# Coder-Yu/SELFRec

Hardware: NVIDIA H100
Metric: XSimGCL yelp2018 train steps/sec (higher is better)
Workload: dtype f32

## Files before the change

include/selfrec_b200.h:

```cpp
#ifndef SELFREC_B200_H
#define SELFREC_B200_H

#include <stdint.h>

#ifdef __cplusplus
extern "C" {
#endif

#define SRB_OK 0
#define SRB_ERR_ARG (-1)
#define SRB_ERR_CUDA (-2)
#define SRB_ERR_STATE (-3)

const char* srb_last_error(void);
int srb_version(void);
int64_t srb_launch_count(void);
int srb_device_ok(void);

#define SRB_HUB_CHUNK 2048
#define SRB_HUB_MIN_NNZ 4096
#define SRB_HUB_WARP_SEG 256
typedef struct srb_hub_split {
  int32_t n_rows;
  int32_t n_work;
  const int32_t* first;
  const int32_t* work;
  float* part;
  const int32_t* seg;
  const int32_t* seg_cnt;
  const int32_t* order_cta;
  const int32_t* order_warp;
  int32_t n_cta;
  int32_t n_warp;
} srb_hub_split;

typedef struct srb_spmm_desc {
  const int32_t* rowptr;
  const int32_t* colidx;
  const float* vals;
  int32_t n_rows;
  int32_t n_cols;
  int32_t d;
  const int32_t* row_order;
  int32_t n_long_rows;
  int32_t n_vlong_rows;
  srb_hub_split hub;
  const int32_t* n_vlong_dev;
  const uint32_t* col_mask;
  const float* X;
// ... 3 lines not shown
  int32_t noise_mode;
  const float* noise;
  float eps;
  uint64_t philox_seed;
  uint64_t philox_offset;
  const int32_t* philox_step_dev;
  const float* sum_in;
  float* sum_out;
  float sum_scale;
  float* adam_p;
  float* adam_m;
  float* adam_v;
  const float* adam_scalars;
  double beta1, beta2;
  float adam_eps;
} srb_spmm_desc;

int srb_spmm_csr(const srb_spmm_desc* desc, void* stream);
int srb_spmm_epilogue_rows(const srb_spmm_desc* desc, void* stream);

typedef struct srb_encoder_desc {
  const int32_t* rowptr;
  const int32_t* colidx;
  const float* vals;
  const int32_t* row_order;
  int32_t n_long_rows;
  int32_t n_vlong_rows;
  srb_hub_split hub;
  int32_t n;
  int32_t d;
// ... 5 lines not shown
  float eps;
  uint64_t philox_seed;
  uint64_t philox_offset;
  const int32_t* philox_step_dev;
  const int32_t* last_rows;
  int32_t n_last_rows;
  const int32_t* last_rows_nv_dev;
  srb_hub_split last_rows_hub;
  float* last_rows_out;
  const float* E0;
  float* final_out;
  float* cl_out;
  float* work0;
  float* work1;
  const float* x1;
} srb_encoder_desc;

int srb_encoder_forward(const srb_encoder_desc* desc, void* stream);

typedef struct srb_bpr_desc {
  const float* emb;
  const float* l2_emb;
  int32_t n_users;
  int32_t d;
  const int32_t* u_idx;
  const int32_t* i_idx;
  const int32_t* j_idx;
  const int32_t* b_dev;
  int32_t b;
  float emb_scale;
// ... 138 lines not shown

int srb_rank_hit_masks(const int32_t* topk_ids, int32_t n_q, int32_t k, const int32_t* users,
                       const int32_t* test_ptr, const int32_t* test_idx, uint64_t* hit_mask,
                       void* stream);

enum { SRB_MODEL_MF = 0, SRB_MODEL_LIGHTGCN = 1, SRB_MODEL_SIMGCL = 2, SRB_MODEL_XSIMGCL = 3, SRB_MODEL_SGL = 4 };

typedef struct srb_graph_csr {
  const int32_t* rowptr;
  const int32_t* colidx;
  const float* vals;
  const int32_t* row_order;
  int32_t n_long_rows;
  int32_t n_vlong_rows;
  srb_hub_split hub;
} srb_graph_csr;

typedef struct srb_step_desc {
  int32_t model;
  int32_t n_users, n_items, d, n_layers;
  int32_t batch_cap;
  int32_t layer_cl;
  float eps, tau, cl_rate;
  float reg;
  double lr, beta1, beta2;
  float adam_eps;
  float l2_div;
  int32_t noise_mode;
  const float* noise;
  uint64_t philox_seed;
// ... 118 lines not shown
```

selfrec_b200/_lib.py:

```python
import ctypes as C
import os

HERE = os.path.dirname(os.path.abspath(__file__))
LIB_PATH = os.path.join(HERE, "libselfrec_b200.so")

c_i32p = C.POINTER(C.c_int32)
c_f32p = C.POINTER(C.c_float)
c_u32p = C.POINTER(C.c_uint32)
c_i64p = C.POINTER(C.c_int64)
VP = C.c_void_p


class SrbError(RuntimeError):
    pass


class HubSplit(C.Structure):
    _fields_ = [("n_rows", C.c_int32), ("n_work", C.c_int32), ("first", VP), ("work", VP), ("part", VP), ("seg", VP), ("seg_cnt", VP),
                ("order_cta", VP), ("order_warp", VP), ("n_cta", C.c_int32), ("n_warp", C.c_int32)]


HUB_CHUNK = 2048
HUB_MIN_NNZ = 4096
HUB_WARP_SEG = 256


class SpmmDesc(C.Structure):
    _fields_ = [
        ("rowptr", VP), ("colidx", VP), ("vals", VP),
        ("n_rows", C.c_int32), ("n_cols", C.c_int32), ("d", C.c_int32),
        ("row_order", VP), ("n_long_rows", C.c_int32), ("n_vlong_rows", C.c_int32), ("hub", HubSplit), ("n_vlong_dev", VP), ("col_mask", VP), ("X", VP), ("Y", VP), ("extra", VP), ("extra_scale", C.c_float),
        ("noise_mode", C.c_int32), ("noise", VP), ("eps", C.c_float),
        ("philox_seed", C.c_uint64), ("philox_offset", C.c_uint64), ("philox_step_dev", VP),
        ("sum_in", VP), ("sum_out", VP), ("sum_scale", C.c_float),
        ("adam_p", VP), ("adam_m", VP), ("adam_v", VP), ("adam_scalars", VP),
        ("beta1", C.c_double), ("beta2", C.c_double), ("adam_eps", C.c_float),
    ]


class EncoderDesc(C.Structure):
    _fields_ = [
        ("rowptr", VP), ("colidx", VP), ("vals", VP), ("row_order", VP), ("n_long_rows", C.c_int32),
        ("n_vlong_rows", C.c_int32), ("hub", HubSplit), ("n", C.c_int32), ("d", C.c_int32), ("n_layers", C.c_int32), ("include_ego", C.c_int32),
        ("layer_cl", C.c_int32), ("noise_mode", C.c_int32), ("noise", VP), ("eps", C.c_float),
        ("philox_seed", C.c_uint64), ("philox_offset", C.c_uint64), ("philox_step_dev", VP),
        ("last_rows", VP), ("n_last_rows", C.c_int32), ("last_rows_nv_dev", VP), ("last_rows_hub", HubSplit), ("last_rows_out", VP),
        ("E0", VP), ("final_out", VP), ("cl_out", VP), ("work0", VP), ("work1", VP), ("x1", VP),
    ]


class ScatterSeg(C.Structure):
    _fields_ = [("src", VP), ("rows", VP), ("n_dev", VP), ("n", C.c_int32), ("row_off", C.c_int32), ("scale", C.c_float)]


class BprDesc(C.Structure):
    _fields_ = [
        ("emb", VP), ("l2_emb", VP), ("n_users", C.c_int32), ("d", C.c_int32),
        ("u_idx", VP), ("i_idx", VP), ("j_idx", VP), ("b_dev", VP), ("b", C.c_int32),
        ("emb_scale", C.c_float), ("reg", C.c_float), ("l2_terms", C.c_int32), ("l2_div", C.c_float),
        ("grad_scale", C.c_float), ("losses", VP), ("g_emb", VP), ("g_l2", VP), ("scratch", VP),
    ]

# ... 12 lines not shown
        ("prob", InfoNceProblem * 4), ("workspace", VP), ("workspace_bytes", C.c_int64),
    ]


class TopkDesc(C.Structure):
    _fields_ = [
        ("user_emb", VP), ("item_emb", VP), ("n_items", C.c_int32), ("d", C.c_int32),
        ("users", VP), ("n_q", C.c_int32), ("rated_ptr", VP), ("rated_idx", VP), ("k", C.c_int32),
        ("out_ids", VP), ("out_scores", VP), ("impl", C.c_int32), ("workspace", VP),
        ("workspace_bytes", C.c_int64),
    ]


class GraphCsr(C.Structure):
    _fields_ = [("rowptr", VP), ("colidx", VP), ("vals", VP), ("row_order", VP), ("n_long_rows", C.c_int32), ("n_vlong_rows", C.c_int32),
                ("hub", HubSplit)]


class GraphAssembleDesc(C.Structure):
    _fields_ = [
        ("n_users", C.c_int32), ("n_items", C.c_int32), ("nnz", C.c_int64), ("ui_ptr", VP), ("ui_col", VP), ("ui_val", VP),
        ("iu_ptr", VP), ("iu_col", VP), ("iu_perm", VP), ("keep_flags", VP), ("keep_idx", VP), ("n_keep", C.c_int64),
        ("reset_weights", C.c_int32), ("dinv_table", VP), ("dinv_table_n", C.c_int32), ("rowptr", VP), ("colidx", VP),
        ("vals", VP), ("dinv", VP), ("out_cap", C.c_int64), ("nnz_out", VP), ("workspace", VP), ("workspace_bytes", C.c_int64),
    ]


class StepDesc(C.Structure):
    _fields_ = [
        ("model", C.c_int32), ("n_users", C.c_int32), ("n_items", C.c_int32), ("d", C.c_int32),
        ("n_layers", C.c_int32), ("batch_cap", C.c_int32), ("layer_cl", C.c_int32),
# ... 141 lines not shown
```

selfrec_b200/csrc/engine.cu:

```cuda
#include <stdlib.h>
#include <algorithm>
#include <mutex>
#include "spmm_args.cuh"

namespace srb {

static bool pdl_enabled() {
  static const bool on = [] {
    const char* e = getenv("SRB_PDL");
    return !(e && e[0] == '0');
  }();
  return on;
}

static thread_local bool t_pdl = false;
bool pdl_active() { return t_pdl; }

struct PdlScope {
  PdlScope() { t_pdl = pdl_enabled(); }
  ~PdlScope() { t_pdl = false; }
};

struct Ws {
  float* final_;
// ... 352 lines not shown
static ScatterSeg seg(const float* src, const int32_t* rows, const int32_t* n_dev, int n, int row_off, float scale) {
  ScatterSeg g = {src, rows, n_dev, n, row_off, scale};
  return g;
}

static int encoder(const srb_step_desc* s, const Ws& w, const srb_graph_csr* g, bool include_ego, int noise_mode, int view,
                   int layer_cl, float* final_out, float* cl_out, cudaStream_t st, const float* x1 = nullptr) {
  srb_encoder_desc e = {};
  e.rowptr = g->rowptr;
  e.colidx = g->colidx;
  e.vals = g->vals;
  e.row_order = g->row_order;
  e.n_long_rows = g->n_long_rows;
  e.n_vlong_rows = g->n_vlong_rows;
  e.hub = g->hub;
  e.n = s->n_users + s->n_items;
  e.d = s->d;
  e.n_layers = s->n_layers;
  e.include_ego = include_ego;
  e.layer_cl = layer_cl;
  e.noise_mode = noise_mode;
  if (noise_mode == 1) e.noise = s->noise + (size_t)view * s->n_layers * e.n * e.d;
  e.eps = s->eps;
  e.philox_seed = s->philox_seed;
  e.philox_offset = noise_offset(view, 0);
  e.philox_step_dev = s->step_dev;
  e.E0 = s->params;
  if (cl_out && layer_cl == s->n_layers) {
    e.final_out = final_out;
  } else {
// ... 152 lines not shown
```

selfrec_b200/csrc/spmm.cu:

```cuda
#include "spmm_args.cuh"

namespace srb {

__device__ __forceinline__ void st4_cs(float* p, const float4& v, int stream) {
  if (stream) __stcs(reinterpret_cast<float4*>(p), v);
  else st4(p, v);
}

__device__ __forceinline__ void st4_peer(float* p, const float4& v, int mc) {
  if (mc) asm volatile("multimem.st.weak.global.v4.f32 [%0], {%1, %2, %3, %4};" ::"l"(p), "f"(v.x), "f"(v.y), "f"(v.z), "f"(v.w) : "memory");
  else st4(p, v);
}

__device__ __forceinline__ float4 ldg4_if(const float* p, bool pred) {
  float4 r = f4_zero();
  asm("{\n\t.reg .pred q;\n\tsetp.ne.b32 q, %5, 0;\n\t@q ld.global.nc.v4.f32 {%0, %1, %2, %3}, [%4];\n\t}"
      : "+f"(r.x), "+f"(r.y), "+f"(r.z), "+f"(r.w)
      : "l"(p), "r"((int)pred));
  return r;
}

template <int D>
__device__ __forceinline__ void spmm_epilogue(const SpmmArgs& a, int row, int gl, float4 acc0, float4 acc1, bool valid) {
  constexpr int LPR = D / 8;
  constexpr int HALF = D / 2;
  {
    if (a.stage_peer[0]) {
      if (!valid) return;
      int o = 0;
#pragma unroll 1
      while (row >= a.stage_bounds[o + 1]) ++o;
      float* dst = a.stage_peer[o] + ((size_t)a.stage_rank * a.stage_cap + (row - a.stage_bounds[o])) * D + gl * 4;
      st4(dst, acc0);
      st4(dst + HALF, acc1);
// ... 93 lines not shown
  p4.F = p4.F - step_size * (m.F / (sqrtf(v4.F) / bc2_sqrt + a.aeps));
        SRB_ADAM1(x) SRB_ADAM1(y) SRB_ADAM1(z) SRB_ADAM1(w)
#undef SRB_ADAM1
        st4(a.ap + o2, p4);
        st4_cs(a.am + o2, m, a.stream);
        st4_cs(a.av + o2, v4, a.stream);
        if (a.world > 0 && a.peer_p[0]) {
#pragma unroll 1
          for (int g = 0; g < a.world; ++g) st4_peer(a.peer_p[g] + o2, p4, a.peer_mc);
        }
      }
    }
  }
}

template <int D, bool MASKED>
__device__ __forceinline__ void spmm_gather(const SpmmArgs& a, int p, int end, int stride, int gl, float4& acc0, float4& acc1) {
  constexpr int LPR = D / 8;
  constexpr int HALF = D / 2;
  constexpr int SB = LPR < 4 ? LPR : 4;
  constexpr bool masked = MASKED;
  const int lane = threadIdx.x & 31;
  const int gbase = lane - gl;
  int c = 0;
  float v = 0.f;
  bool hit = false;
  if (p + gl < end) {
    c = a.stream ? __ldcs(a.colidx + p + gl) : __ldg(a.colidx + p + gl);
    v = a.stream ? __ldcs(a.vals + p + gl) : __ldg(a.vals + p + gl);
    if (masked) hit = (__ldg(a.col_mask + (c >> 5)) >> (c & 31)) & 1u;
  }
  while (__any_sync(SRB_FULL_MASK, p < end)) {
    int cn = 0;
    float vn = 0.f;
    bool hitn = false;
    if (p + stride + gl < end) {
      cn = a.stream ? __ldcs(a.colidx + p + stride + gl) : __ldg(a.colidx + p + stride + gl);
      vn = a.stream ? __ldcs(a.vals + p + stride + gl) : __ldg(a.vals + p + stride + gl);
      if (masked) hitn = (__ldg(a.col_mask + (cn >> 5)) >> (cn & 31)) & 1u;
    }
    if (!masked) {
#pragma unroll
      for (int j0 = 0; j0 < LPR; j0 += SB) {
        if (j0 > 0 && !__any_sync(SRB_FULL_MASK, p + j0 < end)) break;
        float vv[SB];
        float4 x0[SB], x1[SB];
#pragma unroll
        for (int j = 0; j < SB; ++j) {
          const int cc = __shfl_sync(SRB_FULL_MASK, c, j0 + j, LPR);
          vv[j] = __shfl_sync(SRB_FULL_MASK, v, j0 + j, LPR);
          const float* xr = a.X + (size_t)cc * D + gl * 4;
          x0[j] = ldg4(xr);
          x1[j] = ldg4(xr + HALF);
        }
// ... 16 lines not shown
          gm &= gm - 1;
          const int cc = __shfl_sync(SRB_FULL_MASK, c, gbase + src);
          const float vs = __shfl_sync(SRB_FULL_MASK, v, gbase + src);
          vv[j] = live ? vs : 0.f;
          const float* xr = a.X + (size_t)cc * D + gl * 4;
          x0[j] = ldg4_if(xr, live);
          x1[j] = ldg4_if(xr + HALF, live);
        }
#pragma unroll
        for (int j = 0; j < SB; ++j) {
          acc0 = f4_fma(vv[j], x0[j], acc0);
          acc1 = f4_fma(vv[j], x1[j], acc1);
        }
      }
    }
    c = cn;
    v = vn;
    hit = hitn;
    p += stride;
  }
}

__device__ __forceinline__ void xor_reduce_groups(float4& acc0, float4& acc1, int lpr) {
  for (int o = lpr; o < 32; o <<= 1) {
    acc0.x += __shfl_xor_sync(SRB_FULL_MASK, acc0.x, o);
    acc0.y += __shfl_xor_sync(SRB_FULL_MASK, acc0.y, o);
    acc0.z += __shfl_xor_sync(SRB_FULL_MASK, acc0.z, o);
    acc0.w += __shfl_xor_sync(SRB_FULL_MASK, acc0.w, o);
    acc1.x += __shfl_xor_sync(SRB_FULL_MASK, acc1.x, o);
    acc1.y += __shfl_xor_sync(SRB_FULL_MASK, acc1.y, o);
    acc1.z += __shfl_xor_sync(SRB_FULL_MASK, acc1.z, o);
    acc1.w += __shfl_xor_sync(SRB_FULL_MASK, acc1.w, o);
  }
}

template <int D, bool MASKED>
__global__ void __launch_bounds__(256) spmm_hub_kernel(const SpmmArgs a) {
  constexpr int LPR = D / 8;
  const int lane = threadIdx.x & 31;
  const int wib = threadIdx.x >> 5;
  const int grp = lane / LPR;
  const int gl = lane % LPR;
  pdl_wait();
  pdl_trigger();
  const int n_work = a.seg ? a.n_cta : (a.n_vlong_dev ? min(a.n_vlong_dev[4], a.n_work) : a.n_work);
  __shared__ float4 part[8][2][LPR];
  for (int k = blockIdx.x; k < n_work; k += gridDim.x) {
    int w = k, beg, end;
    if (a.seg) {
      w = __ldg(a.order_cta + k);
      beg = __ldg(a.seg + 2 * w);
      end = __ldg(a.seg + 2 * w + 1);
    } else {
      const int row = __ldg(a.hub_work + 2 * w);
      const int ci = __ldg(a.hub_work + 2 * w + 1);
      const int rbeg = __ldg(a.rowptr + row), rend = __ldg(a.rowptr + row + 1);
      beg = min(rend, rbeg + ci * SRB_HUB_CHUNK);
      end = min(rend, beg + SRB_HUB_CHUNK);
    }
    const int per = ((end - beg + 255) / 256) * 32;
    const int wbeg = beg + wib * per;
    const int wend = min(end, wbeg + per);
    float4 acc0 = f4_zero(), acc1 = f4_zero();
    spmm_gather<D, MASKED>(a, wbeg + grp * LPR, wend, 32, gl, acc0, acc1);
    xor_reduce_groups(acc0, acc1, LPR);
    if (grp == 0) {
      part[wib][0][gl] = acc0;
      part[wib][1][gl] = acc1;
    }
    __syncthreads();
    if (wib == 0 && grp == 0) {
      acc0 = f4_zero();
      acc1 = f4_zero();
#pragma unroll
      for (int q = 0; q < 8; ++q) {
        acc0 = f4_add(acc0, part[q][0][gl]);
        acc1 = f4_add(acc1, part[q][1][gl]);
      }
      float* dst = a.hub_part + (size_t)w * D + gl * 4;
// ... 6 lines not shown

template <int D, bool MASKED>
__global__ void __launch_bounds__(256) spmm_seg_warp_kernel(const SpmmArgs a) {
  constexpr int LPR = D / 8;
  const int lane = threadIdx.x & 31;
  const int grp = lane / LPR;
  const int gl = lane % LPR;
  const int warp0 = (blockIdx.x * blockDim.x + threadIdx.x) >> 5;
  const int nwarps = (gridDim.x * blockDim.x) >> 5;
  pdl_wait();
  pdl_trigger();
  for (int k = warp0; k < a.n_warp; k += nwarps) {
    const int w = __ldg(a.order_warp + k);
    const int beg = __ldg(a.seg + 2 * w), end = __ldg(a.seg + 2 * w + 1);
    float4 acc0 = f4_zero(), acc1 = f4_zero();
    spmm_gather<D, MASKED>(a, beg + grp * LPR, end, 32, gl, acc0, acc1);
    xor_reduce_groups(acc0, acc1, LPR);
    if (grp == 0) {
      float* dst = a.hub_part + (size_t)w * D + gl * 4;
      st4(dst, acc0);
      st4(dst + D / 2, acc1);
    }
  }
}

template <int D>
__global__ void __launch_bounds__(256) spmm_hub_finish_kernel(const SpmmArgs a) {
  constexpr int LPR = D / 8;
  constexpr int RPW = 32 / LPR;
  const int lane = threadIdx.x & 31;
  const int grp = lane / LPR;
// ... 8 lines not shown
    const int row = __ldg(a.row_order + vr);
    const int first = __ldg(a.hub_first + vr);
    const int deg = __ldg(a.rowptr + row + 1) - __ldg(a.rowptr + row);
    const int nch = a.seg ? __ldg(a.seg_cnt + vr) : (deg + SRB_HUB_CHUNK - 1) / SRB_HUB_CHUNK;
    float4 acc0 = f4_zero(), acc1 = f4_zero();
    for (int c = grp; c < nch; c += RPW) {
      const float* src = a.hub_part + (size_t)(first + c) * D + gl * 4;
      acc0 = f4_add(acc0, *reinterpret_cast<const float4*>(src));
      acc1 = f4_add(acc1, *reinterpret_cast<const float4*>(src + D / 2));
    }
    xor_reduce_groups(acc0, acc1, LPR);
    spmm_epilogue<D>(a, row, gl, acc0, acc1, grp == 0);
  }
}

template <int D, bool MASKED>
__global__ void __launch_bounds__(256) spmm_csr_kernel(const SpmmArgs a) {
  constexpr int LPR = D / 8;
  constexpr int RPW = 32 / LPR;
  const int lane = threadIdx.x & 31;
  const int wib = threadIdx.x >> 5;
  const int grp = lane / LPR;
  const int gl = lane % LPR;
  const int warp0 = (blockIdx.x * blockDim.x + threadIdx.x) >> 5;
  const int nwarps = (gridDim.x * blockDim.x) >> 5;

  pdl_wait();
  pdl_trigger();
  peer_wait(a.ps);
  int n_vlong = a.n_vlong, n_long = a.n_long, n_short = a.n_rows - a.n_huge - a.n_vlong - a.n_long;
  const int32_t* ro_v = a.row_order ? a.row_order + a.n_huge : nullptr;
  const int32_t* ro_l = a.row_order ? ro_v + n_vlong : nullptr;
// ... 3 lines not shown
    n_vlong = min(a.n_vlong_dev[1], a.n_rows);
    n_long = min(a.n_vlong_dev[2], a.n_rows);
    n_short = min(a.n_vlong_dev[3], a.n_rows);
    ro_v = a.row_order + a.n_rows;
    ro_l = a.row_order + 2 * a.n_rows;
    ro_s = a.row_order + 3 * a.n_rows;
  }
  __shared__ float4 part[8][2][LPR];
  for (int vr = blockIdx.x; vr < n_vlong; vr += gridDim.x) {
    const int row = ro_v ? __ldg(ro_v + vr) : vr;
    const int beg = __ldg(a.rowptr + row);
    const int end = __ldg(a.rowptr + row + 1);
    const int per = ((end - beg + 255) / 256) * 32;
    const int wbeg = beg + wib * per;
    const int wend = min(end, wbeg + per);
    float4 acc0 = f4_zero(), acc1 = f4_zero();
    spmm_gather<D, MASKED>(a, wbeg + grp * LPR, wend, 32, gl, acc0, acc1);
    xor_reduce_groups(acc0, acc1, LPR);
    if (grp == 0) {
      part[wib][0][gl] = acc0;
      part[wib][1][gl] = acc1;
    }
    __syncthreads();
    if (wib == 0) {
      acc0 = f4_zero();
      acc1 = f4_zero();
#pragma unroll
      for (int w = 0; w < 8; ++w) {
        acc0 = f4_add(acc0, part[w][0][gl]);
        acc1 = f4_add(acc1, part[w][1][gl]);
      }
      spmm_epilogue<D>(a, row, gl, acc0, acc1, grp == 0);
    }
    __syncthreads();
  }

  const int n_items = n_long + (n_short + RPW - 1) / RPW;
  for (int item = warp0; item < n_items; item += nwarps) {
    const bool is_long = item < n_long;
    const int k = is_long ? item : (item - n_long) * RPW + grp;
    bool valid = is_long || k < n_short;
    int row = 0, p = 0, end = 0;
    if (valid) {
      if (is_long) row = ro_l ? __ldg(ro_l + k) : id_l + k;
      else row = ro_s ? __ldg(ro_s + k) : id_s + k;
      p = __ldg(a.rowptr + row);
      end = __ldg(a.rowptr + row + 1);
    }
    if (is_long) p += grp * LPR;
    float4 acc0 = f4_zero(), acc1 = f4_zero();
    spmm_gather<D, MASKED>(a, p, end, is_long ? 32 : LPR, gl, acc0, acc1);
    if (is_long) {
      xor_reduce_groups(acc0, acc1, LPR);
      valid = valid && grp == 0;
    }
    spmm_epilogue<D>(a, row, gl, acc0, acc1, valid);
  }
  peer_signal(a.ps);
}

__device__ __forceinline__ float4 multimem_ld_reduce_add4(const float* mc) {
  float4 v;
  asm volatile("multimem.ld_reduce.relaxed.sys.global.add.v4.f32 {%0, %1, %2, %3}, [%4];"
               : "=f"(v.x), "=f"(v.y), "=f"(v.z), "=f"(v.w)
               : "l"(mc)
               : "memory");
  return v;
}

template <int D>
__global__ void __launch_bounds__(256) reduce_rows_kernel(const SpmmArgs a, const ReduceArgs r) {
  constexpr int LPR = D / 8;
  constexpr int RPW = 32 / LPR;
// ... 117 lines not shown
  long long blocks = ((long long)(r.n_slice + rpw - 1) / rpw + 7) / 8;
  const long long cap = (long long)sm_count() * (r.small_grid ? 1 : 8);
  if (blocks > cap) blocks = cap;
  if (blocks < 1) blocks = 1;
  switch (d) {
    case 16: reduce_rows_kernel<16><<<(int)blocks, 256, 0, st>>>(a, r); break;
    case 32: reduce_rows_kernel<32><<<(int)blocks, 256, 0, st>>>(a, r); break;
    case 64: reduce_rows_kernel<64><<<(int)blocks, 256, 0, st>>>(a, r); break;
    case 128: reduce_rows_kernel<128><<<(int)blocks, 256, 0, st>>>(a, r); break;
    case 256: reduce_rows_kernel<256><<<(int)blocks, 256, 0, st>>>(a, r); break;
    default: set_error("reduce_rows: unsupported d=%d (16, 32, 64, 128, 256)", d); return SRB_ERR_ARG;
  }
  return post_launch("reduce_rows_kernel");
}

template <int D, bool M>
static int launch_spmm_dma(const SpmmArgs& a, int hub_blocks, int blocks, cudaStream_t st) {
  if (hub_blocks > 0) {
    if (a.seg && a.n_warp > 0) {
      const int wb = max(1, min((a.n_warp + 7) / 8, blocks));
      SRB_TRY(launch_kernel(spmm_seg_warp_kernel<D, M>, wb, 256, 0, st, "spmm_seg_warp_kernel", a));
    }
    SRB_TRY(launch_kernel(spmm_hub_kernel<D, M>, hub_blocks, 256, 0, st, "spmm_hub_kernel", a));
    const int nh = a.n_vlong_dev ? a.n_rows : a.n_huge;
    SRB_TRY(launch_kernel(spmm_hub_finish_kernel<D>, max(1, min((nh + 7) / 8, hub_blocks)), 256, 0, st, "spmm_hub_finish_kernel", a));
  }
  return launch_kernel(spmm_csr_kernel<D, M>, blocks, 256, 0, st, "spmm_csr_kernel", a);
}

template <int D>
static int launch_spmm_d(const SpmmArgs& a, int hub_blocks, int blocks, cudaStream_t st) {
  if (a.col_mask != nullptr) return launch_spmm_dma<D, true>(a, hub_blocks, blocks, st);
  return launch_spmm_dma<D, false>(a, hub_blocks, blocks, st);
}

int launch_spmm(const SpmmArgs& a, int d, cudaStream_t st) {
  if (a.n_rows == 0) return SRB_OK;
  const int threads = 256;
  const int rpw = 32 / (d / 8);
  const long long items = (long long)a.n_long + ((long long)a.n_rows - a.n_huge - a.n_vlong - a.n_long + rpw - 1) / rpw;
  long long blocks = (items + threads / 32 - 1) / (threads / 32);
  if (a.n_vlong_dev) blocks = ((long long)a.n_rows + threads / 32 - 1) / (threads / 32);
  if (blocks < a.n_vlong) blocks = a.n_vlong;
  const long long cap = (long long)sm_count() * 8;
  if (blocks > cap) blocks = cap;
  if (blocks < 1) blocks = 1;
  long long hub_blocks = a.seg ? (a.n_cta > 0 ? a.n_cta : (a.n_work > 0 ? 1 : 0)) : a.n_work;
  if (hub_blocks > cap) hub_blocks = cap;
// ... 26 lines not shown
  SRB_REQUIRE(!hub || d->hub.n_rows <= d->n_rows, "spmm: more split rows than rows");
  a.n_huge = (hub && !a.n_vlong_dev) ? d->hub.n_rows : 0;
  a.hub_first = hub ? d->hub.first : nullptr;
  a.hub_work = hub ? d->hub.work : nullptr;
  a.hub_part = hub ? d->hub.part : nullptr;
  a.n_work = hub ? d->hub.n_work : 0;
  const bool segs = hub && !a.n_vlong_dev && d->hub.seg != nullptr;
  SRB_REQUIRE(!segs || (d->hub.seg_cnt && (d->hub.n_cta == 0 || d->hub.order_cta) && (d->hub.n_warp == 0 || d->hub.order_warp)),
              "spmm: column-blocked split-row lists incomplete");
  a.seg = segs ? d->hub.seg : nullptr;
  a.seg_cnt = segs ? d->hub.seg_cnt : nullptr;
  a.order_cta = segs ? d->hub.order_cta : nullptr;
  a.order_warp = segs ? d->hub.order_warp : nullptr;
  a.n_cta = segs ? d->hub.n_cta : 0;
  a.n_warp = segs ? d->hub.n_warp : 0;
  const int rest = d->n_rows - a.n_huge;
  a.n_vlong = (d->row_order && d->n_vlong_rows > 0) ? (d->n_vlong_rows < rest ? d->n_vlong_rows : rest) : 0;
  a.col_mask = d->col_mask;
  a.n_long = (d->row_order && d->n_long_rows > 0) ? (d->n_long_rows < rest - a.n_vlong ? d->n_long_rows : rest - a.n_vlong) : 0;
  a.X = d->X;
  a.Y = d->Y;
  a.extra = d->extra;
  a.extra_scale = d->extra_scale;
  a.seed_mask = nullptr;
  a.seed = nullptr;
  a.noise_mode = d->noise_mode;
  a.noise = d->noise;
  a.eps = d->eps;
  a.pkey = make_uint2((uint32_t)d->philox_seed, (uint32_t)(d->philox_seed >> 32));
  a.poff = make_uint2((uint32_t)d->philox_offset, (uint32_t)(d->philox_offset >> 32));
// ... 19 lines not shown
  a.stage_rank = a.stage_cap = 0;
  for (int g = 0; g < 8; ++g) a.peer[g] = a.peer_sum[g] = a.peer_p[g] = a.stage_peer[g] = nullptr;
  for (int g = 0; g < 9; ++g) a.stage_bounds[g] = 0;
  return SRB_OK;
}

int graph_args(const srb_graph_csr& g, int n_rows, int n_cols, int d, const float* X, SpmmArgs& a) {
  srb_spmm_desc p = {};
  p.rowptr = g.rowptr;
  p.colidx = g.colidx;
  p.vals = g.vals;
  p.row_order = g.row_order;
  p.n_long_rows = g.n_long_rows;
  p.n_vlong_rows = g.n_vlong_rows;
  p.hub = g.hub;
  p.n_rows = n_rows;
  p.n_cols = n_cols;
  p.d = d;
  p.X = X;
  p.extra_scale = 1.f;
  p.sum_scale = 1.f;
  return fill_args(&p, a);
}

}

extern "C" int srb_spmm_csr(const srb_spmm_desc* desc, void* stream) {
  srb::SpmmArgs a;
  SRB_TRY(srb::fill_args(desc, a));
  return srb::launch_spmm(a, desc->d, (cudaStream_t)stream);
// ... 47 lines not shown
    for (int j = 0; j < n_src; ++j) live = live && src[j] != py;
    live = live && n_src < 4;
    if (live) src[n_src++] = py;
    px = py;
  }
  const bool batch_mean = last_on_rows && live;
  for (int k = k0; k < L; ++k) {
    srb_spmm_desc s = {};
    s.rowptr = e->rowptr;
    s.colidx = e->colidx;
    s.vals = e->vals;
    s.row_order = e->row_order;
    s.n_long_rows = e->n_long_rows;
    s.n_vlong_rows = e->n_vlong_rows;
    s.hub = e->hub;
    s.n_rows = e->n;
    s.n_cols = e->n;
    s.d = e->d;
    s.X = x;
    const bool last = (k == L - 1);
    float* y = nullptr;
    if (cl_hit && k == e->layer_cl - 1) y = e->cl_out;
    else if (!last) y = (x == e->work0) ? e->work1 : e->work0;
    s.Y = y;
    s.noise_mode = e->noise_mode;
    if (e->noise_mode == 1) s.noise = e->noise + (size_t)k * nd;
    s.eps = e->eps;
    s.philox_seed = e->philox_seed;
    s.philox_offset = e->philox_offset + (uint64_t)k;
    s.philox_step_dev = e->philox_step_dev;
// ... 30 lines not shown
```

selfrec_b200/csrc/spmm_args.cuh:

```cuda
#pragma once
#include "common.cuh"

namespace srb {

struct PeerSync {
  int* flags[8];
  int* epoch;
  int* counter;
  int* err;
  int world, rank;
  int wait, signal;
};

__device__ __forceinline__ void st_release_sys(int* p, int v) { asm volatile("st.release.sys.global.s32 [%0], %1;" ::"l"(p), "r"(v) : "memory"); }
__device__ __forceinline__ int ld_acquire_sys(const int* p) {
  int v;
  asm volatile("ld.acquire.sys.global.s32 %0, [%1];" : "=r"(v) : "l"(p) : "memory");
  return v;
}

__device__ __forceinline__ int ld_relaxed_sys(const int* p) {
  int v;
  asm volatile("ld.relaxed.sys.global.s32 %0, [%1];" : "=r"(v) : "l"(p) : "memory");
  return v;
// ... 24 lines not shown
    __threadfence();
    if (atomicAdd(s.counter, 1) == (int)gridDim.x - 1) {
      *s.counter = 0;
      __threadfence_system();
      const int e = *s.epoch + 1;
      *s.epoch = e;
      for (int q = 0; q < s.world; ++q) st_release_sys(s.flags[q] + s.rank, e);
    }
  }
}

struct SpmmArgs {
  const int32_t* rowptr;
  const int32_t* colidx;
  const float* vals;
  const int32_t* row_order;
  int32_t n_rows;
  const int32_t* n_vlong_dev;
  const uint32_t* col_mask;
  int32_t n_huge;
  int32_t n_vlong;
  int32_t n_long;
  const int32_t* hub_first;
  const int32_t* hub_work;
  int32_t n_work;
  float* hub_part;
  const int32_t* seg;
  const int32_t* seg_cnt;
  const int32_t* order_cta;
  const int32_t* order_warp;
// ... 83 lines not shown
```

selfrec_b200/ops.py:

```python
import ctypes as C

import numpy as np
import torch

from . import _lib
from ._lib import SrbError

_SUPPORTED_D = (16, 32, 64, 128, 256)
LONG_ROW_NNZ = 64
VLONG_ROW_NNZ = 256


def _stream():
    return C.c_void_p(torch.cuda.current_stream().cuda_stream)


def _p(t):
    return None if t is None else C.c_void_p(t.data_ptr())


def _f32c(t, name):
    if not isinstance(t, torch.Tensor):
        raise TypeError(f"{name}: expected a torch.Tensor")
    if not t.is_cuda:
# ... 66 lines not shown
    src = torch.repeat_interleave(torch.arange(ukey.numel(), device=dev), pieces, output_size=n_seg)
    sub = torch.arange(n_seg, device=dev) - torch.repeat_interleave(torch.cumsum(pieces, 0) - pieces, pieces, output_size=n_seg)
    b = sbeg[src] + sub * _lib.HUB_CHUNK
    e = torch.minimum(b + _lib.HUB_CHUNK, sbeg[src] + cnt[src])
    srow = ukey[src] // nblk
    sblk = ukey[src] % nblk
    per_row = torch.bincount(srow, minlength=n_rows)
    first = torch.cumsum(per_row, 0) - per_row
    order = torch.sort(sblk * n_rows + srow, stable=True).indices
    long_seg = (e - b)[order] > _lib.HUB_WARP_SEG
    i32 = lambda t: t.to(torch.int32).contiguous()
    return dict(seg=i32(torch.stack([b, e], 1)), first=i32(first), cnt=i32(per_row), order_cta=i32(order[long_seg]),
                order_warp=i32(order[~long_seg]), n_seg=n_seg, block_cols=W)


class SparseAdj:

    def __init__(self, mat):
        import scipy.sparse as sp

        csr = sp.csr_matrix(mat, dtype=np.float32)
        csr.sort_indices()
        if csr.nnz >= 2**31:
            raise SrbError("SparseAdj: nnz must fit in int32")
        self._csr = csr
        self.shape = tuple(csr.shape)
        self.nnz = int(csr.nnz)
        self.device = torch.device("cpu")
        self.rowptr = self.colidx = self.vals = self.row_order = None
        self.n_long = self.n_vlong = self.n_huge = self.n_work = 0
        self.hub_first = self.hub_work = None
        self._hub_part = {}
        self._t = None
        self._symmetric = None

    @classmethod
    def from_device(cls, rowptr, colidx, vals, shape, symmetric=None, classes=None):
        self = cls.__new__(cls)
        self._csr = None
        self.shape = tuple(int(x) for x in shape)
        self.nnz = int(colidx.numel())
        self.device = rowptr.device
        self.rowptr, self.colidx, self.vals = rowptr, colidx, vals
        self._hub_part = {}
        self._t = None
        self._symmetric = symmetric
        self._set_classes(classify_rows(rowptr) if classes is None else classes)
        return self

    def _set_classes(self, c):
        self.row_order = c["row_order"]
        self.n_huge, self.n_vlong, self.n_long = c["n_huge"], c["n_vlong"], c["n_long"]
        self.hub_first, self.hub_work, self.n_work = c["hub_first"], c["hub_work"], c["n_work"]

    def cuda(self, device=None):
        _lib.require_device()
        dev = torch.device("cuda", torch.cuda.current_device() if device is None else device) if not isinstance(device, torch.device) else device
        if self.rowptr is not None and self.device == dev:
            return self
        if self._csr is None:
            raise SrbError("SparseAdj.from_device handles stay on the device they were built on")
        csr = self._csr
        self.rowptr = torch.from_numpy(csr.indptr.astype(np.int32)).to(dev)
        self.colidx = torch.from_numpy(csr.indices.astype(np.int32)).to(dev)
        self.vals = torch.from_numpy(csr.data.astype(np.float32)).to(dev)
        self._set_classes(classify_rows(self.rowptr))
        self._hub_part = {}
        self.device = dev
        return self

    def to(self, device):
        device = torch.device(device)
        if device.type != "cuda":
            raise SrbError("SparseAdj lives on a CUDA device (no CPU fallback)")
        return self.cuda(device)

    def size(self, dim=None):
        return self.shape if dim is None else self.shape[dim]

    def _nnz(self):
# ... 48 lines not shown
                h.n_work, h.first = segs["n_seg"], _p(segs["first"])
                h.seg, h.seg_cnt = _p(segs["seg"]), _p(segs["cnt"])
                h.order_cta, h.order_warp = _p(segs["order_cta"]), _p(segs["order_warp"])
                h.n_cta, h.n_warp = int(segs["order_cta"].numel()), int(segs["order_warp"].numel())
                h.work = _p(self.hub_work)
            else:
                h.n_work, h.first, h.work = self.n_work, _p(self.hub_first), _p(self.hub_work)
        return h

    def graph_struct(self, d):
        g = _lib.GraphCsr()
        g.rowptr, g.colidx, g.vals, g.row_order = _p(self.rowptr), _p(self.colidx), _p(self.vals), _p(self.row_order)
        g.n_long_rows = self.n_long
        g.n_vlong_rows = self.n_vlong
        g.hub = self.hub_struct(d)
        return g


def _spmm_raw(adj, x, y=None, _entry="srb_spmm_csr", **epi):
    lib = _lib.require_device()
    if adj.rowptr is None:
        adj.cuda(x.device)
    n_rows, n_cols = adj.shape
    d = x.shape[1]
    if x.shape[0] != n_cols:
        raise ValueError(f"spmm: A is {adj.shape} but X has {x.shape[0]} rows")
    if d not in _SUPPORTED_D:
        raise SrbError(f"spmm: embedding size {d} unsupported (16, 32, 64, 128, 256)")
    desc = _lib.SpmmDesc()
    desc.rowptr, desc.colidx, desc.vals = _p(adj.rowptr), _p(adj.colidx), _p(adj.vals)
    desc.row_order = _p(adj.row_order)
    desc.n_long_rows, desc.n_vlong_rows = adj.n_long, adj.n_vlong
    desc.hub = adj.hub_struct(d)
    desc.n_rows, desc.n_cols, desc.d = n_rows, n_cols, d
    desc.X = _p(x)
    desc.Y = _p(y)
    desc.extra_scale = 1.0
    desc.sum_scale = 1.0
    keep = []
    for k, v in epi.items():
        if isinstance(v, torch.Tensor):
            keep.append(v)
            setattr(desc, k, _p(v))
        else:
            setattr(desc, k, v)
    _lib.check(getattr(lib, _entry)(C.byref(desc), _stream()), _entry)


# ... 23 lines not shown

def encoder_forward(adj, e0, n_layers, include_ego, noise=None, eps=0.0, layer_cl=0, philox_seed=None, want_cl=False):
    lib = _lib.require_device()
    e0 = _f32c(e0, "encoder E0")
    if adj.rowptr is None:
        adj.cuda(e0.device)
    n, d = e0.shape
    final = torch.empty_like(e0)
    cl = torch.empty_like(e0) if want_cl else None
    w0 = torch.empty_like(e0)
    w1 = torch.empty_like(e0)
    desc = _lib.EncoderDesc()
    desc.rowptr, desc.colidx, desc.vals, desc.row_order = _p(adj.rowptr), _p(adj.colidx), _p(adj.vals), _p(adj.row_order)
    desc.n_long_rows, desc.n_vlong_rows = adj.n_long, adj.n_vlong
    desc.hub = adj.hub_struct(d)
    desc.n, desc.d, desc.n_layers, desc.include_ego, desc.layer_cl = n, d, n_layers, int(include_ego), int(layer_cl)
    if noise is not None:
        noise = _f32c(noise, "encoder noise")
        if tuple(noise.shape) != (n_layers, n, d):
            raise ValueError("encoder noise must be [n_layers, N, d]")
        desc.noise_mode, desc.noise = 1, _p(noise)
    elif philox_seed is not None:
        desc.noise_mode, desc.philox_seed = 2, int(philox_seed)
    desc.eps = float(eps)
    desc.E0, desc.final_out, desc.cl_out, desc.work0, desc.work1 = _p(e0), _p(final), _p(cl), _p(w0), _p(w1)
    _lib.check(lib.srb_encoder_forward(C.byref(desc), _stream()), "srb_encoder_forward")
    return final, cl


class _BprFn(torch.autograd.Function):
# ... 375 lines not shown
```

Measured before the change: 1909.

## Pack CSR column index and degree into one word to halve SpMM index traffic

Builds a packed adjacency in which each nonzero is a single 32-bit word holding the column index and the column's degree. The value is rebuilt on the fly as the product of inverse-sqrt-degree table entries for row and column. The pack is used only when it reproduces the original values bitwise. This cuts per-nonzero index/value loads from 8 bytes to 4 in the SpMM gather, at the cost of an extra cached table lookup and a multiply per nonzero. A packed CSR kernel variant with launch bounds of 4 blocks per SM is added.

After: 1978 (median of 6 runs). +3.6%, better.

```diff
diff --git a/include/selfrec_b200.h b/include/selfrec_b200.h
--- a/include/selfrec_b200.h
+++ b/include/selfrec_b200.h
@@ -33,6 +33,12 @@
   int32_t n_cta;
   int32_t n_warp;
 } srb_hub_split;
+
+typedef struct srb_csr_pack {
+  const uint32_t* word;
+  const float* dtab;
+  int32_t cbits;
+} srb_csr_pack;
 
 typedef struct srb_spmm_desc {
   const int32_t* rowptr;
@@ -66,6 +72,7 @@
   const float* adam_scalars;
   double beta1, beta2;
   float adam_eps;
+  srb_csr_pack pack;
 } srb_spmm_desc;
 
 int srb_spmm_csr(const srb_spmm_desc* desc, void* stream);
@@ -101,6 +108,7 @@
   float* work0;
   float* work1;
   const float* x1;
+  srb_csr_pack pack;
 } srb_encoder_desc;
 
 int srb_encoder_forward(const srb_encoder_desc* desc, void* stream);
@@ -269,6 +277,7 @@
   int32_t n_long_rows;
   int32_t n_vlong_rows;
   srb_hub_split hub;
+  srb_csr_pack pack;
 } srb_graph_csr;
 
 typedef struct srb_step_desc {
diff --git a/selfrec_b200/_lib.py b/selfrec_b200/_lib.py
--- a/selfrec_b200/_lib.py
+++ b/selfrec_b200/_lib.py
@@ -23,6 +23,10 @@
 HUB_CHUNK = 2048
 HUB_MIN_NNZ = 4096
 HUB_WARP_SEG = 256
+
+
+class CsrPack(C.Structure):
+    _fields_ = [("word", VP), ("dtab", VP), ("cbits", C.c_int32)]
 
 
 class SpmmDesc(C.Structure):
@@ -34,7 +38,7 @@
         ("philox_seed", C.c_uint64), ("philox_offset", C.c_uint64), ("philox_step_dev", VP),
         ("sum_in", VP), ("sum_out", VP), ("sum_scale", C.c_float),
         ("adam_p", VP), ("adam_m", VP), ("adam_v", VP), ("adam_scalars", VP),
-        ("beta1", C.c_double), ("beta2", C.c_double), ("adam_eps", C.c_float),
+        ("beta1", C.c_double), ("beta2", C.c_double), ("adam_eps", C.c_float), ("pack", CsrPack),
     ]
 
 
@@ -45,7 +49,7 @@
         ("layer_cl", C.c_int32), ("noise_mode", C.c_int32), ("noise", VP), ("eps", C.c_float),
         ("philox_seed", C.c_uint64), ("philox_offset", C.c_uint64), ("philox_step_dev", VP),
         ("last_rows", VP), ("n_last_rows", C.c_int32), ("last_rows_nv_dev", VP), ("last_rows_hub", HubSplit), ("last_rows_out", VP),
-        ("E0", VP), ("final_out", VP), ("cl_out", VP), ("work0", VP), ("work1", VP), ("x1", VP),
+        ("E0", VP), ("final_out", VP), ("cl_out", VP), ("work0", VP), ("work1", VP), ("x1", VP), ("pack", CsrPack),
     ]
 
 
@@ -88,7 +92,7 @@
 
 class GraphCsr(C.Structure):
     _fields_ = [("rowptr", VP), ("colidx", VP), ("vals", VP), ("row_order", VP), ("n_long_rows", C.c_int32), ("n_vlong_rows", C.c_int32),
-                ("hub", HubSplit)]
+                ("hub", HubSplit), ("pack", CsrPack)]
 
 
 class GraphAssembleDesc(C.Structure):
diff --git a/selfrec_b200/csrc/engine.cu b/selfrec_b200/csrc/engine.cu
--- a/selfrec_b200/csrc/engine.cu
+++ b/selfrec_b200/csrc/engine.cu
@@ -390,6 +390,7 @@
   e.n_long_rows = g->n_long_rows;
   e.n_vlong_rows = g->n_vlong_rows;
   e.hub = g->hub;
+  e.pack = g->pack;
   e.n = s->n_users + s->n_items;
   e.d = s->d;
   e.n_layers = s->n_layers;
diff --git a/selfrec_b200/csrc/spmm.cu b/selfrec_b200/csrc/spmm.cu
--- a/selfrec_b200/csrc/spmm.cu
+++ b/selfrec_b200/csrc/spmm.cu
@@ -18,6 +18,21 @@
       : "+f"(r.x), "+f"(r.y), "+f"(r.z), "+f"(r.w)
       : "l"(p), "r"((int)pred));
   return r;
+}
+
+__device__ __forceinline__ void ld_pair(const SpmmArgs& a, int i, int& c, float& v) {
+  c = a.stream ? __ldcs(a.colidx + i) : __ldg(a.colidx + i);
+#ifdef SRB_PROBE_NO_VALS
+  v = 0.03125f;
+#else
+  v = a.stream ? __ldcs(a.vals + i) : __ldg(a.vals + i);
+#endif
+}
+
+__device__ __forceinline__ uint32_t ld_word(const SpmmArgs& a, int i) { return a.stream ? __ldcs(a.pk + i) : __ldg(a.pk + i); }
+__device__ __forceinline__ void unpack_word(const SpmmArgs& a, uint32_t w, float dr, int& c, float& v) {
+  c = (int)(w & ((1u << a.cbits) - 1u));
+  v = __fmul_rn(dr, __ldg(a.dtab + (w >> a.cbits)));
 }
 
 template <int D>
@@ -141,8 +156,8 @@
   }
 }
 
-template <int D, bool MASKED>
-__device__ __forceinline__ void spmm_gather(const SpmmArgs& a, int p, int end, int stride, int gl, float4& acc0, float4& acc1) {
+template <int D, bool MASKED, bool PACKED>
+__device__ __forceinline__ void spmm_gather(const SpmmArgs& a, int p, int end, int stride, int gl, float dr, float4& acc0, float4& acc1) {
   constexpr int LPR = D / 8;
   constexpr int HALF = D / 2;
   constexpr int SB = LPR < 4 ? LPR : 4;
@@ -153,18 +168,23 @@
   float v = 0.f;
   bool hit = false;
   if (p + gl < end) {
-    c = a.stream ? __ldcs(a.colidx + p + gl) : __ldg(a.colidx + p + gl);
-    v = a.stream ? __ldcs(a.vals + p + gl) : __ldg(a.vals + p + gl);
+    if (PACKED) unpack_word(a, ld_word(a, p + gl), dr, c, v);
+    else ld_pair(a, p + gl, c, v);
     if (masked) hit = (__ldg(a.col_mask + (c >> 5)) >> (c & 31)) & 1u;
   }
   while (__any_sync(SRB_FULL_MASK, p < end)) {
     int cn = 0;
     float vn = 0.f;
     bool hitn = false;
-    if (p + stride + gl < end) {
-      cn = a.stream ? __ldcs(a.colidx + p + stride + gl) : __ldg(a.colidx + p + stride + gl);
-      vn = a.stream ? __ldcs(a.vals + p + stride + gl) : __ldg(a.vals + p + stride + gl);
-      if (masked) hitn = (__ldg(a.col_mask + (cn >> 5)) >> (cn & 31)) & 1u;
+    uint32_t wn = 0;
+    const bool more = p + stride + gl < end;
+    if (more) {
+      if (PACKED) {
+        wn = ld_word(a, p + stride + gl);
+      } else {
+        ld_pair(a, p + stride + gl, cn, vn);
+        if (masked) hitn = (__ldg(a.col_mask + (cn >> 5)) >> (cn & 31)) & 1u;
+      }
     }
     if (!masked) {
 #pragma unroll
@@ -211,6 +231,10 @@
         }
       }
     }
+    if (PACKED && more) {
+      unpack_word(a, wn, dr, cn, vn);
+      if (masked) hitn = (__ldg(a.col_mask + (cn >> 5)) >> (cn & 31)) & 1u;
+    }
     c = cn;
     v = vn;
     hit = hitn;
@@ -231,7 +255,7 @@
   }
 }
 
-template <int D, bool MASKED>
+template <int D, bool MASKED, bool PACKED>
 __global__ void __launch_bounds__(256) spmm_hub_kernel(const SpmmArgs a) {
   constexpr int LPR = D / 8;
   const int lane = threadIdx.x & 31;
@@ -244,6 +268,7 @@
   __shared__ float4 part[8][2][LPR];
   for (int k = blockIdx.x; k < n_work; k += gridDim.x) {
     int w = k, beg, end;
+    float dr = 0.f;
     if (a.seg) {
       w = __ldg(a.order_cta + k);
       beg = __ldg(a.seg + 2 * w);
@@ -254,12 +279,13 @@
       const int rbeg = __ldg(a.rowptr + row), rend = __ldg(a.rowptr + row + 1);
       beg = min(rend, rbeg + ci * SRB_HUB_CHUNK);
       end = min(rend, beg + SRB_HUB_CHUNK);
+      if (PACKED) dr = __ldg(a.dtab + (rend - rbeg));
     }
     const int per = ((end - beg + 255) / 256) * 32;
     const int wbeg = beg + wib * per;
     const int wend = min(end, wbeg + per);
     float4 acc0 = f4_zero(), acc1 = f4_zero();
-    spmm_gather<D, MASKED>(a, wbeg + grp * LPR, wend, 32, gl, acc0, acc1);
+    spmm_gather<D, MASKED, PACKED>(a, wbeg + grp * LPR, wend, 32, gl, dr, acc0, acc1);
     xor_reduce_groups(acc0, acc1, LPR);
     if (grp == 0) {
       part[wib][0][gl] = acc0;
@@ -296,7 +322,7 @@
     const int w = __ldg(a.order_warp + k);
     const int beg = __ldg(a.seg + 2 * w), end = __ldg(a.seg + 2 * w + 1);
     float4 acc0 = f4_zero(), acc1 = f4_zero();
-    spmm_gather<D, MASKED>(a, beg + grp * LPR, end, 32, gl, acc0, acc1);
+    spmm_gather<D, MASKED, false>(a, beg + grp * LPR, end, 32, gl, 0.f, acc0, acc1);
     xor_reduce_groups(acc0, acc1, LPR);
     if (grp == 0) {
       float* dst = a.hub_part + (size_t)w * D + gl * 4;
@@ -335,8 +361,8 @@
   }
 }
 
-template <int D, bool MASKED>
-__global__ void __launch_bounds__(256) spmm_csr_kernel(const SpmmArgs a) {
+template <int D, bool MASKED, bool PACKED>
+__device__ __forceinline__ void spmm_csr_body(const SpmmArgs& a) {
   constexpr int LPR = D / 8;
   constexpr int RPW = 32 / LPR;
   const int lane = threadIdx.x & 31;
@@ -370,8 +396,9 @@
     const int per = ((end - beg + 255) / 256) * 32;
     const int wbeg = beg + wib * per;
     const int wend = min(end, wbeg + per);
+    const float dr = PACKED ? __ldg(a.dtab + (end - beg)) : 0.f;
     float4 acc0 = f4_zero(), acc1 = f4_zero();
-    spmm_gather<D, MASKED>(a, wbeg + grp * LPR, wend, 32, gl, acc0, acc1);
+    spmm_gather<D, MASKED, PACKED>(a, wbeg + grp * LPR, wend, 32, gl, dr, acc0, acc1);
     xor_reduce_groups(acc0, acc1, LPR);
     if (grp == 0) {
       part[wib][0][gl] = acc0;
@@ -397,15 +424,17 @@
     const int k = is_long ? item : (item - n_long) * RPW + grp;
     bool valid = is_long || k < n_short;
     int row = 0, p = 0, end = 0;
+    float dr = 0.f;
     if (valid) {
       if (is_long) row = ro_l ? __ldg(ro_l + k) : id_l + k;
       else row = ro_s ? __ldg(ro_s + k) : id_s + k;
       p = __ldg(a.rowptr + row);
       end = __ldg(a.rowptr + row + 1);
+      if (PACKED) dr = __ldg(a.dtab + (end - p));
     }
     if (is_long) p += grp * LPR;
     float4 acc0 = f4_zero(), acc1 = f4_zero();
-    spmm_gather<D, MASKED>(a, p, end, is_long ? 32 : LPR, gl, acc0, acc1);
+    spmm_gather<D, MASKED, PACKED>(a, p, end, is_long ? 32 : LPR, gl, dr, acc0, acc1);
     if (is_long) {
       xor_reduce_groups(acc0, acc1, LPR);
       valid = valid && grp == 0;
@@ -413,6 +442,16 @@
     spmm_epilogue<D>(a, row, gl, acc0, acc1, valid);
   }
   peer_signal(a.ps);
+}
+
+template <int D, bool MASKED>
+__global__ void __launch_bounds__(256) spmm_csr_kernel(const SpmmArgs a) {
+  spmm_csr_body<D, MASKED, false>(a);
+}
+
+template <int D, bool MASKED>
+__global__ void __launch_bounds__(256, 4) spmm_csr_packed_kernel(const SpmmArgs a) {
+  spmm_csr_body<D, MASKED, true>(a);
 }
 
 __device__ __forceinline__ float4 multimem_ld_reduce_add4(const float* mc) {
@@ -560,24 +599,29 @@
   return post_launch("reduce_rows_kernel");
 }
 
-template <int D, bool M>
+template <int D, bool M, bool P>
 static int launch_spmm_dma(const SpmmArgs& a, int hub_blocks, int blocks, cudaStream_t st) {
   if (hub_blocks > 0) {
     if (a.seg && a.n_warp > 0) {
       const int wb = max(1, min((a.n_warp + 7) / 8, blocks));
       SRB_TRY(launch_kernel(spmm_seg_warp_kernel<D, M>, wb, 256, 0, st, "spmm_seg_warp_kernel", a));
     }
-    SRB_TRY(launch_kernel(spmm_hub_kernel<D, M>, hub_blocks, 256, 0, st, "spmm_hub_kernel", a));
+    SRB_TRY(launch_kernel(spmm_hub_kernel<D, M, P>, hub_blocks, 256, 0, st, "spmm_hub_kernel", a));
     const int nh = a.n_vlong_dev ? a.n_rows : a.n_huge;
     SRB_TRY(launch_kernel(spmm_hub_finish_kernel<D>, max(1, min((nh + 7) / 8, hub_blocks)), 256, 0, st, "spmm_hub_finish_kernel", a));
   }
+  if (P) return launch_kernel(spmm_csr_packed_kernel<D, M>, blocks, 256, 0, st, "spmm_csr_packed_kernel", a);
   return launch_kernel(spmm_csr_kernel<D, M>, blocks, 256, 0, st, "spmm_csr_kernel", a);
 }
 
 template <int D>
 static int launch_spmm_d(const SpmmArgs& a, int hub_blocks, int blocks, cudaStream_t st) {
-  if (a.col_mask != nullptr) return launch_spmm_dma<D, true>(a, hub_blocks, blocks, st);
-  return launch_spmm_dma<D, false>(a, hub_blocks, blocks, st);
+  if (a.pk != nullptr) {
+    if (a.col_mask != nullptr) return launch_spmm_dma<D, true, true>(a, hub_blocks, blocks, st);
+    return launch_spmm_dma<D, false, true>(a, hub_blocks, blocks, st);
+  }
+  if (a.col_mask != nullptr) return launch_spmm_dma<D, true, false>(a, hub_blocks, blocks, st);
+  return launch_spmm_dma<D, false, false>(a, hub_blocks, blocks, st);
 }
 
 int launch_spmm(const SpmmArgs& a, int d, cudaStream_t st) {
@@ -634,6 +678,12 @@
   a.order_warp = segs ? d->hub.order_warp : nullptr;
   a.n_cta = segs ? d->hub.n_cta : 0;
   a.n_warp = segs ? d->hub.n_warp : 0;
+  const bool packed = d->pack.word != nullptr && !segs;
+  SRB_REQUIRE(!packed || (d->pack.dtab && d->pack.cbits >= 1 && d->pack.cbits <= 31 && (long long)d->n_cols <= (1ll << d->pack.cbits)),
+              "spmm: incomplete packed adjacency");
+  a.pk = packed ? d->pack.word : nullptr;
+  a.dtab = packed ? d->pack.dtab : nullptr;
+  a.cbits = packed ? d->pack.cbits : 0;
   const int rest = d->n_rows - a.n_huge;
   a.n_vlong = (d->row_order && d->n_vlong_rows > 0) ? (d->n_vlong_rows < rest ? d->n_vlong_rows : rest) : 0;
   a.col_mask = d->col_mask;
@@ -683,6 +733,7 @@
   p.n_long_rows = g.n_long_rows;
   p.n_vlong_rows = g.n_vlong_rows;
   p.hub = g.hub;
+  p.pack = g.pack;
   p.n_rows = n_rows;
   p.n_cols = n_cols;
   p.d = d;
@@ -760,6 +811,7 @@
     s.n_long_rows = e->n_long_rows;
     s.n_vlong_rows = e->n_vlong_rows;
     s.hub = e->hub;
+    s.pack = e->pack;
     s.n_rows = e->n;
     s.n_cols = e->n;
     s.d = e->d;
diff --git a/selfrec_b200/csrc/spmm_args.cuh b/selfrec_b200/csrc/spmm_args.cuh
--- a/selfrec_b200/csrc/spmm_args.cuh
+++ b/selfrec_b200/csrc/spmm_args.cuh
@@ -62,6 +62,9 @@
   const int32_t* rowptr;
   const int32_t* colidx;
   const float* vals;
+  const uint32_t* pk;
+  const float* dtab;
+  int32_t cbits;
   const int32_t* row_order;
   int32_t n_rows;
   const int32_t* n_vlong_dev;
diff --git a/selfrec_b200/ops.py b/selfrec_b200/ops.py
--- a/selfrec_b200/ops.py
+++ b/selfrec_b200/ops.py
@@ -104,6 +104,27 @@
                 order_warp=i32(order[~long_seg]), n_seg=n_seg, block_cols=W)
 
 
+def pack_csr(rowptr, colidx, vals, shape):
+    n_rows, n_cols = (int(x) for x in shape)
+    nnz = int(colidx.numel())
+    if n_rows != n_cols or nnz == 0:
+        return None
+    deg = (rowptr[1:] - rowptr[:-1]).to(torch.int64)
+    max_deg = int(deg.max())
+    cbits = max(1, (n_cols - 1).bit_length())
+    if cbits + max_deg.bit_length() > 32:
+        return None
+    from .data.device_graph import dinv_table
+    dtab = torch.from_numpy(dinv_table(max_deg)).to(rowptr.device)
+    col = colidx.to(torch.int64)
+    dc = deg[col]
+    rebuilt = torch.repeat_interleave(dtab[deg], deg, output_size=nnz) * dtab[dc]
+    if not torch.equal(rebuilt.view(torch.int32), vals.contiguous().view(torch.int32)):
+        return None
+    w = col | (dc << cbits)
+    return dict(word=torch.where(w >= 1 << 31, w - (1 << 32), w).to(torch.int32).contiguous(), dtab=dtab, cbits=cbits)
+
+
 class SparseAdj:
 
     def __init__(self, mat):
@@ -117,7 +138,7 @@
         self.shape = tuple(csr.shape)
         self.nnz = int(csr.nnz)
         self.device = torch.device("cpu")
-        self.rowptr = self.colidx = self.vals = self.row_order = None
+        self.rowptr = self.colidx = self.vals = self.row_order = self.pack = None
         self.n_long = self.n_vlong = self.n_huge = self.n_work = 0
         self.hub_first = self.hub_work = None
         self._hub_part = {}
@@ -132,6 +153,7 @@
         self.nnz = int(colidx.numel())
         self.device = rowptr.device
         self.rowptr, self.colidx, self.vals = rowptr, colidx, vals
+        self.pack = None
         self._hub_part = {}
         self._t = None
         self._symmetric = symmetric
@@ -154,6 +176,7 @@
         self.rowptr = torch.from_numpy(csr.indptr.astype(np.int32)).to(dev)
         self.colidx = torch.from_numpy(csr.indices.astype(np.int32)).to(dev)
         self.vals = torch.from_numpy(csr.data.astype(np.float32)).to(dev)
+        self.pack = pack_csr(self.rowptr, self.colidx, self.vals, self.shape)
         self._set_classes(classify_rows(self.rowptr))
         self._hub_part = {}
         self.device = dev
@@ -232,7 +255,14 @@
         g.n_long_rows = self.n_long
         g.n_vlong_rows = self.n_vlong
         g.hub = self.hub_struct(d)
+        g.pack = self.pack_struct()
         return g
+
+    def pack_struct(self):
+        p = _lib.CsrPack()
+        if self.pack is not None:
+            p.word, p.dtab, p.cbits = _p(self.pack["word"]), _p(self.pack["dtab"]), self.pack["cbits"]
+        return p
 
 
 def _spmm_raw(adj, x, y=None, _entry="srb_spmm_csr", **epi):
@@ -250,6 +280,7 @@
     desc.row_order = _p(adj.row_order)
     desc.n_long_rows, desc.n_vlong_rows = adj.n_long, adj.n_vlong
     desc.hub = adj.hub_struct(d)
+    desc.pack = adj.pack_struct()
     desc.n_rows, desc.n_cols, desc.d = n_rows, n_cols, d
     desc.X = _p(x)
     desc.Y = _p(y)
@@ -303,6 +334,7 @@
     desc.rowptr, desc.colidx, desc.vals, desc.row_order = _p(adj.rowptr), _p(adj.colidx), _p(adj.vals), _p(adj.row_order)
     desc.n_long_rows, desc.n_vlong_rows = adj.n_long, adj.n_vlong
     desc.hub = adj.hub_struct(d)
+    desc.pack = adj.pack_struct()
     desc.n, desc.d, desc.n_layers, desc.include_ego, desc.layer_cl = n, d, n_layers, int(include_ego), int(layer_cl)
     if noise is not None:
         noise = _f32c(noise, "encoder noise")
```
